# ALVI-Labs/frankenstein

Measured on AMD Instinct MI355X. Metric: neural frames/sec (train fwd+bwd+AdamW, whole job), higher is better.
Workload: dtype bf16; 1 GPU; brainformer-small (6L d=384 6x64 heads, N=6144 tokens) + 2-block perceiver, L1 head; fwd+bwd+clip+AdamW; per_gpu_batch=32, global_batch=32, frames_T=600, electrodes=256, parallelism=dp1, weights=random-init (seed 42)

## Files before the change

### frankenstein_amd/_lib.py

```python
from __future__ import annotations

import ctypes as C
from pathlib import Path

import os

LIB_PATH = Path(os.environ.get("FRANKEN_HIP_LIB") or Path(__file__).resolve().parent / "libfranken_hip.so")

FK_F32, FK_BF16 = 0, 1
MASK_NONE, MASK_CAUSAL, MASK_BLOCK_CAUSAL, MASK_PREFIX, MASK_KEYPAD, MASK_DENSE = 0, 1, 2, 3, 4, 5
NORM_LAYER, NORM_RMS = 0, 1
ATTN_Q_PRESCALED = 1
GEMV_GELU = 1
NT_RING2, NT_RING192, NT_RING128, NT_BIG, NT_GLDS4, NT_GLDS, NT_STAGED = range(7)
NT_ROUTE_F32 = -2
ATTN_FWD_GENERIC, ATTN_FWD_FEWQ, ATTN_FWD_PS, ATTN_FWD_ASM = range(4)
ATTN_DQ_GENERIC, ATTN_DQ_FEWQ, ATTN_DQ_PS, ATTN_DQ_ASM = range(4)
ATTN_DKDV_GENERIC, ATTN_DKDV_PS, ATTN_DKDV_ASM, ATTN_DKDVW_ASM = range(4)

_p, _i64, _int, _f32, _f64, _sz, _u32 = C.c_void_p, C.c_int64, C.c_int, C.c_float, C.c_double, C.c_size_t, C.c_uint32

SIGNATURES = {
    "fk_version": (_int, []),
    "fk_last_error": (C.c_char_p, []),
    "fk_gemm_nt": (_int, [_p, _i64, _p, _i64, _p, _i64, _i64, _i64, _i64, _p, _p, _i64, _i64, _int, _int, _p]),
    "fk_gemv_nt": (_int, [_p, _i64, _p, _i64, _p, _i64, _i64, _i64, _i64, _p, _p, _i64, _p, _p, _f32, _int, _int, _int, _p]),
    "fk_gemm_nt_rope": (_int, [_p, _i64, _p, _i64, _p, _i64, _i64, _i64, _i64, _p, _p, _i64, _i64, _i64, _i64, _i64, _i64, _i64, _int, _p]),
    "fk_gemm_nt_swiglu": (_int, [_p, _i64, _p, _i64, _p, _i64, _p, _i64, _i64, _i64, _i64, _int, _p]),
    "fk_gemm_nt_dswiglu": (_int, [_p, _i64, _p, _i64, _p, _i64, _p, _i64, _i64, _i64, _i64, _int, _p]),
    "fk_mlp_bwd_fused": (_int, [_p, _i64, _p, _i64, _p, _i64, _p, _i64, _p, _i64, _p, _i64, _i64, _i64, _i64, _int, _p]),
    "fk_gemm_nt_route": (_int, [_i64, _i64, _i64, _int, _int, _int, _int]),
    "fk_gemm_tn_route": (_int, [_i64, _i64, _i64, _int, _p, _p]),
    "fk_gemm_tn_workspace_bytes": (_sz, [_i64, _i64, _i64, _int]),
    "fk_gemm_tn": (_int, [_p, _i64, _p, _i64, _p, _i64, _i64, _i64, _i64, _int, _int, _p, _sz, _p]),
    "fk_gemm_tn_swiglu": (_int, [_p, _i64, _p, _i64, _p, _p, _i64, _i64, _i64, _i64, _int, _p, _sz, _p]),
    "fk_colsum_workspace_bytes": (_sz, [_i64, _i64]),
    "fk_colsum": (_int, [_p, _i64, _p, _i64, _i64, _int, _int, _p, _sz, _p]),
    "fk_attn_fwd": (_int, [_p, _p, _p, _p, _p] + [_i64] * 13 + [_int, _i64, _i64, _i64, _p, _p, _f32, _int, _int, _p]),
    "fk_attn_bwd": (_int, [_p] * 10 + [_i64] * 13 + [_int, _i64, _i64, _i64, _p, _p, _f32, _p, _i64, _i64, _int, _int, _p]),
    "fk_attn_fwd_dropout": (_int, [_p, _p, _p, _p, _p] + [_i64] * 13 + [_int, _i64, _i64, _i64, _p, _p, _f32, _int, _f32, _p, _u32, _int, _p]),
    "fk_attn_bwd_dropout": (_int, [_p] * 10 + [_i64] * 13 + [_int, _i64, _i64, _i64, _p, _p, _f32, _p, _i64, _i64, _int, _f32, _p, _u32, _int, _p]),
    "fk_attn_route": (_int, [_i64, _i64, _i64, _int, _int, _i64, _i64, _i64, _int, _int, _int, _p, _p, _p]),
    "fk_dropout": (_int, [_p, _p, _p, _i64, _f32, _p, _u32, _int, _p]),
    "fk_norm_fwd": (_int, [_p, _p, _p, _p, _p, _p, _i64, _i64, _f32, _int, _int, _p]),
    "fk_norm_bwd_workspace_bytes": (_sz, [_i64, _i64]),
    "fk_norm_bwd": (_int, [_p] * 9 + [_i64, _i64, _int, _int, _int, _p, _sz, _p]),
    "fk_rope": (_int, [_p, _i64, _i64, _i64, _i64, _i64, _p, _i64, _i64, _int, _int, _p]),
    "fk_patchify": (_int, [_p, _p, _i64, _i64, _i64, _i64, _i64, _int, _p]),
    "fk_swiglu_fwd": (_int, [_p, _p, _i64, _i64, _int, _p]),
    "fk_swiglu_bwd": (_int, [_p, _p, _p, _i64, _i64, _int, _p]),
    "fk_gelu_fwd": (_int, [_p, _p, _i64, _int, _p]),
    "fk_gelu_bwd": (_int, [_p, _p, _p, _i64, _int, _p]),
    "fk_cast_pack": (_int, [_p, _i64, _p, _i64, _i64, _i64, _int, _int, _p]),
    "fk_cast_pack_rows": (_int, [_p, _i64, _p, _i64, _i64, _i64, _int, _i64, _i64, _i64, _int, _p]),
    "fk_cast_pack_multi": (_int, [_p, _i64, _i64, _int, _p]),
    "fk_cast": (_int, [_p, _int, _p, _int, _i64, _p]),
    "fk_add": (_int, [_p, _p, _p, _i64, _int, _p]),
    "fk_gather_rows": (_int, [_p, _i64, _int, _p, _i64, _p, _i64, _int, _i64, _i64, _i64, _int, _p]),
    "fk_scatter_add_rows": (_int, [_p, _int, _p, _i64, _p, _i64, _i64, _p]),
    "fk_prefix_mask": (_int, [_p, _p, _i64, _p, _p, _i64, _i64, _i64, _p]),
    "fk_copy2d": (_int, [_p, _i64, _p, _i64, _i64, _i64, _int, _p]),
    "fk_attn_combine": (_int, [_p, _p, _p, _p, _i64, _i64, _i64, _i64, _i64, _int, _p]),
    "fk_add2d": (_int, [_p, _i64, _p, _i64, _i64, _i64, _p]),
    "fk_gpt_embed_step": (_int, [_p, _p, _p, _p, _p, _i64, _i64, _i64, _int, _p]),
    "fk_kv_append": (_int, [_p, _p, _p, _i64, _i64, _i64, _int, _p]),
    "fk_attn_decode": (_int, [_p, _i64, _p, _i64, _i64, _p, _i64, _p, _i64, _i64, _i64, _f32, _int, _p]),
    "fk_sample_topk": (_int, [_p, _i64, _i64, _i64, _f32, _i64, _p, _p, _p, _p, _p, _i64, _i64, _p, _p]),
    "fk_attn_decode_beam": (_int, [_p, _i64, _p, _i64, _i64, _p, _i64, _p, _i64, _p, _i64, _i64, _i64, _f32, _int, _p]),
    "fk_beam_topk": (_int, [_p, _i64, _i64, _i64, _f32, _i64, _p, _p, _p]),
    "fk_beam_select": (_int, [_p, _p, _i64, _i64, _i64, _p, _p, _p, _p, _p, _p, _p, _p, _i64, _p, _i64, _p]),
    "fk_attn_decode_beam_grouped": (_int, [_p, _i64, _p, _i64, _i64, _i64, _p, _i64, _p, _i64, _p, _i64, _i64, _i64, _i64, _f32, _int, _int, _p]),
    "fk_beam_select_grouped": (_int, [_p, _p, _i64, _i64, _i64, _i64, _i64, _p, _p, _p, _p, _p, _p, _p, _p, _i64, _p, _i64, _p, _p]),
    "fk_beam_select_eos": (_int, [_p, _p, _i64, _i64, _i64, _i64, _i64, _p, _p, _p, _p, _p, _p, _p, _p, _i64, _p, _i64, _p, _i64, _p, _p, _p, _i64, _p, _p, _p]),
    "fk_beam_backtrack": (_int, [_p, _p, _i64, _i64, _i64, _p, _p, _p, _p, _i64, _p, _i64, _i64, _i64, _i64, _p, _p, _p]),
    "fk_sample_topk_eos": (_int, [_p, _i64, _i64, _i64, _f32, _i64, _p, _p, _p, _p, _p, _i64, _i64, _p, _i64, _p, _p, _p, _p, _p]),
    "fk_sample_topp": (_int, [_p, _i64, _i64, _i64, _f32, _i64, _f32, _p, _p, _p, _p, _p, _i64, _i64, _p, _i64, _p, _p, _p, _p, _p]),
    "fk_logit_rules": (_int, [_p, _i64, _i64, _i64, _f32, _i64, _i64, _i64, _p, _p, _p, _p, _i64, _i64, _i64, _p, _i64, _i64, _int, _p]),
    "fk_im2col1d": (_int, [_p, _p, _i64, _i64, _i64, _i64, _i64, _i64, _int, _p]),
    "fk_col2im1d": (_int, [_p, _p, _i64, _i64, _i64, _i64, _i64, _i64, _int, _p]),
    "fk_elu_fwd": (_int, [_p, _p, _i64, _int, _p]),
    "fk_elu_bwd": (_int, [_p, _p, _p, _i64, _int, _p]),
    "fk_argmax_rows": (_int, [_p, _i64, _p, _i64, _i64, _int, _p]),
    "fk_block_stats_workspace_bytes": (_sz, [_i64, _i64]),
    "fk_block_stats": (_int, [_p, _p, _p, _i64, _i64, _i64, _p, _p, _p, _sz, _p]),
    "fk_zscore_smooth_pad": (_int, [_p, _p, _p, _p, _p, _p, _i64, _i64, _i64, _f64, _p]),
    "fk_gpt_embed_fwd": (_int, [_p, _p, _p, _p, _p, _i64, _i64, _i64, _i64, _i64, _int, _p]),
    "fk_gpt_embed_bwd_wte": (_int, [_p, _p, _p, _i64, _i64, _i64, _i64, _i64, _int, _p]),
    "fk_loss_workspace_bytes": (_sz, [_i64]),
    "fk_l1_loss_fwd": (_int, [_p, _p, _p, _i64, _int, _p, _i64, _int, _p, _sz, _p]),
    "fk_l1_loss_bwd": (_int, [_p, _p, _p, _p, _i64, _int, _p, _i64, _p, _int, _p]),
    "fk_head_ce_workspace_bytes": (_sz, [_i64, _i64]),
    "fk_head_ce_fwd": (_int, [_p, _i64, _p, _i64, _i64, _p, _p, _p, _p, _p, _i64, _i64, _i64, _int, _p, _sz, _p]),
    "fk_head_ce_bwd": (_int, [_p, _i64, _p, _i64, _i64, _p, _p, _p, _p, _p, _p, _i64, _i64, _i64, _p, _i64, _i64, _i64, _i64, _int, _p]),
    "fk_transpose2d": (_int, [_p, _i64, _p, _i64, _i64, _i64, _int, _p]),
    "fk_ce_workspace_bytes": (_sz, [_i64]),
    "fk_ce_loss_fwd": (_int, [_p, _i64, _p, _p, _p, _i64, _i64, _i64, _int, _p, _sz, _p]),
    "fk_ce_loss_bwd": (_int, [_p, _i64, _p, _p, _p, _p, _p, _i64, _i64, _i64, _i64, _int, _p]),
# ... 51 lines not shown
```

### frankenstein_amd/csrc/norm.hip

```cpp
#include <type_traits>

#include "fk_common.h"

namespace {

#ifndef FK_NT_STORES_NORM
#define FK_NT_STORES_NORM 0
#endif
template <typename T> using VIO = VecIO<T, FK_NT_STORES_NORM != 0>;

template <typename T>
__global__ __launch_bounds__(256) void norm_fwd_kernel(const T* x, const float* gamma, const float* beta, T* y,
                                                        float* mean, float* rstd, int64_t rows, int dim, float eps, int kind) {
  constexpr int N = VIO<T>::N;
  const int lane = threadIdx.x & 63, wave = threadIdx.x >> 6;
  const int64_t wstride = (int64_t)gridDim.x * 4;
  for (int64_t row = (int64_t)blockIdx.x * 4 + wave; row < rows; row += wstride) {
    const T* xr = x + row * dim;
    float s = 0.0f;
    float v[N];
    if (kind == FK_NORM_LAYER) {
      for (int c = lane * N; c < dim; c += 64 * N) {
        VIO<T>::load(xr + c, v);
#pragma unroll
        for (int i = 0; i < N; ++i) s += v[i];
      }
    }
    const float mu = kind == FK_NORM_LAYER ? wave_sum(s) / dim : 0.0f;
    float q = 0.0f;
    for (int c = lane * N; c < dim; c += 64 * N) {
      VIO<T>::load(xr + c, v);
#pragma unroll
      for (int i = 0; i < N; ++i) q += (v[i] - mu) * (v[i] - mu);
    }
    const float rs = rsqrtf(wave_sum(q) / dim + eps);
    if (lane == 0) {
      if (mean) mean[row] = mu;
      rstd[row] = rs;
    }
    T* yr = y + row * dim;
    for (int c = lane * N; c < dim; c += 64 * N) {
      VIO<T>::load(xr + c, v);
      float o[N];
#pragma unroll
      for (int i = 0; i < N; ++i) {
        float t = (v[i] - mu) * rs;
        if (kind == FK_NORM_RMS && sizeof(T) == 2) t = (float)(bf16_t)t;
        o[i] = t * gamma[c + i] + (beta ? beta[c + i] : 0.0f);
      }
      VIO<T>::store(yr + c, o);
    }
  }
}

template <int LPR> FK_DEV float row_sum(float v) {
#pragma unroll
  for (int o = LPR / 2; o > 0; o >>= 1) v += __shfl_xor(v, o, 64);
  return v;
}
template <typename T, int LPR, int MAXIT> struct RowFrame {
  static constexpr int N = VIO<T>::N, RPW = 64 / LPR;
  const int l = (threadIdx.x & 63) % LPR, sub = (threadIdx.x & 63) / LPR;
  FK_DEV int col(int it) const { return l * N + it * LPR * N; }
  FK_DEV void load_param(const float* p, bool in, int it, float (&v)[N]) const {
#pragma unroll
    for (int i = 0; i < N; i += 4) {
      const f32x4 p4 = in ? *reinterpret_cast<const f32x4*>(p + col(it) + i) : f32x4{0.0f, 0.0f, 0.0f, 0.0f};
#pragma unroll
      for (int e = 0; e < 4; ++e) v[i + e] = p4[e];
    }
  }
};
template <typename T, int LPR, int MAXIT>
__global__ __launch_bounds__(256) void norm_fwd_fast_kernel(const T* x, const float* gamma, const float* beta, T* y,
                                                             float* mean, float* rstd, int64_t rows, int dim, float eps, int kind) {
  using Frame = RowFrame<T, LPR, MAXIT>;
  constexpr int N = Frame::N, RPW = Frame::RPW;
  const Frame f{};
  const int wave = threadIdx.x >> 6;
  float gm[MAXIT][N], bt[MAXIT][N];
#pragma unroll
  for (int it = 0; it < MAXIT; ++it) {
    const bool in = f.col(it) < dim;
    f.load_param(gamma, in, it, gm[it]);
    f.load_param(beta, in && beta, it, bt[it]);
  }
  const float inv = 1.0f / dim;
  const int64_t stride = (int64_t)gridDim.x * 4 * RPW;
  for (int64_t base = ((int64_t)blockIdx.x * 4 + wave) * RPW; base < rows; base += stride) {
    const int64_t row = base + f.sub;
    const bool ok = row < rows;
    float v[MAXIT][N];
    float s = 0.0f;
#pragma unroll
    for (int it = 0; it < MAXIT; ++it) {
      const int c = f.col(it);
      if (ok && c < dim) VIO<T>::load(x + row * dim + c, v[it]);
      else {
#pragma unroll
        for (int i = 0; i < N; ++i) v[it][i] = 0.0f;
      }
#pragma unroll
      for (int i = 0; i < N; ++i) s += v[it][i];
    }
    const float mu = kind == FK_NORM_LAYER ? row_sum<LPR>(s) * inv : 0.0f;
    float q = 0.0f;
#pragma unroll
    for (int it = 0; it < MAXIT; ++it) {
#pragma unroll
      for (int i = 0; i < N; ++i) {
        const float d = (f.col(it) + i < dim) ? v[it][i] - mu : 0.0f;
        q += d * d;
      }
    }
    const float rs = rsqrtf(row_sum<LPR>(q) * inv + eps);
    if (ok) {
      if (f.l == 0) {
        if (mean) mean[row] = mu;
        rstd[row] = rs;
      }
#pragma unroll
      for (int it = 0; it < MAXIT; ++it) {
        if (f.col(it) < dim) {
          float o[N];
#pragma unroll
          for (int i = 0; i < N; ++i) {
            float t = (v[it][i] - mu) * rs;
            if (kind == FK_NORM_RMS && sizeof(T) == 2) t = (float)(bf16_t)t;
            o[i] = t * gm[it][i] + bt[it][i];
          }
          VIO<T>::store(y + row * dim + f.col(it), o);
        }
      }
    }
  }
}

template <typename T>
__global__ __launch_bounds__(256) void norm_bwd_dx_kernel(const T* dy, const T* x, const float* gamma, const float* mean,
                                                           const float* rstd, const T* dres, T* dx, int64_t rows, int dim, int kind) {
  constexpr int N = VIO<T>::N;
  const int lane = threadIdx.x & 63, wave = threadIdx.x >> 6;
  const int64_t wstride = (int64_t)gridDim.x * 4;
  for (int64_t row = (int64_t)blockIdx.x * 4 + wave; row < rows; row += wstride) {
    const T* xr = x + row * dim;
    const T* gr = dy + row * dim;
    const float mu = (kind == FK_NORM_LAYER) ? mean[row] : 0.0f, rs = rstd[row];
    float s1 = 0.0f, s2 = 0.0f;
    float xv[N], gv[N];
    for (int c = lane * N; c < dim; c += 64 * N) {
      VIO<T>::load(xr + c, xv);
      VIO<T>::load(gr + c, gv);
#pragma unroll
      for (int i = 0; i < N; ++i) {
        const float dg = gv[i] * gamma[c + i];
        s1 += dg;
        s2 += dg * (xv[i] - mu) * rs;
      }
    }
    const float c1 = (kind == FK_NORM_LAYER) ? wave_sum(s1) / dim : 0.0f;
    const float c2 = wave_sum(s2) / dim;
    for (int c = lane * N; c < dim; c += 64 * N) {
      VIO<T>::load(xr + c, xv);
      VIO<T>::load(gr + c, gv);
      float o[N], rv[N];
      if (dres) VIO<T>::load(dres + row * dim + c, rv);
#pragma unroll
      for (int i = 0; i < N; ++i) {
        const float xh = (xv[i] - mu) * rs;
        o[i] = rs * (gv[i] * gamma[c + i] - c1 - xh * c2) + (dres ? rv[i] : 0.0f);
      }
      VIO<T>::store(dx + row * dim + c, o);
    }
  }
}

template <typename T, int LPR, int MAXIT>
__global__ __launch_bounds__(256) void norm_bwd_fused_kernel(const T* dy, const T* x, const float* gamma, const float* mean,
                                                              const float* rstd, const T* dres, T* dx, float* part,
                                                              int64_t rows, int dim, int kind) {
  using Frame = RowFrame<T, LPR, MAXIT>;
  constexpr int N = Frame::N, RPW = Frame::RPW;
  extern __shared__ float red[];
  const Frame f{};
  const int wave = threadIdx.x >> 6;
  float ag[MAXIT][N] = {}, ab[MAXIT][N] = {}, gm[MAXIT][N];
#pragma unroll
  for (int it = 0; it < MAXIT; ++it) f.load_param(gamma, f.col(it) < dim, it, gm[it]);
  const float inv = 1.0f / dim;
  const int64_t stride = (int64_t)gridDim.x * 4 * RPW;
  for (int64_t base = ((int64_t)blockIdx.x * 4 + wave) * RPW; base < rows; base += stride) {
    const int64_t row = base + f.sub;
    const bool ok = row < rows;
    const float mu = (ok && kind == FK_NORM_LAYER) ? mean[row] : 0.0f, rs = ok ? rstd[row] : 0.0f;
    float xv[MAXIT][N], gv[MAXIT][N], rv[MAXIT][N];
    float s1 = 0.0f, s2 = 0.0f;
#pragma unroll
    for (int it = 0; it < MAXIT; ++it) {
      const int c = f.col(it);
      if (ok && c < dim) {
        VIO<T>::load(x + row * dim + c, xv[it]);
        VIO<T>::load(dy + row * dim + c, gv[it]);
        if (dres) VIO<T>::load(dres + row * dim + c, rv[it]);
      } else {
#pragma unroll
        for (int i = 0; i < N; ++i) { xv[it][i] = mu; gv[it][i] = 0.0f; }
      }
#pragma unroll
      for (int i = 0; i < N; ++i) {
        xv[it][i] = (xv[it][i] - mu) * rs;
        const float dg = gv[it][i] * gm[it][i];
        s1 += dg;
        s2 += dg * xv[it][i];
      }
    }
    const float c1 = (kind == FK_NORM_LAYER) ? row_sum<LPR>(s1) * inv : 0.0f;
    const float c2 = row_sum<LPR>(s2) * inv;
#pragma unroll
    for (int it = 0; it < MAXIT; ++it) {
      if (ok && f.col(it) < dim) {
        float o[N];
#pragma unroll
        for (int i = 0; i < N; ++i) {
          o[i] = rs * (gv[it][i] * gm[it][i] - c1 - xv[it][i] * c2) + (dres ? rv[it][i] : 0.0f);
          ag[it][i] += gv[it][i] * xv[it][i];
          ab[it][i] += gv[it][i];
        }
        VIO<T>::store(dx + row * dim + f.col(it), o);
      }
    }
  }
  if (part == nullptr) return;
#pragma unroll
  for (int it = 0; it < MAXIT; ++it)
#pragma unroll
    for (int i = 0; i < N; ++i) {
#pragma unroll
      for (int o = LPR; o < 64; o <<= 1) {
        ag[it][i] += __shfl_xor(ag[it][i], o, 64);
        ab[it][i] += __shfl_xor(ab[it][i], o, 64);
      }
    }
  if (f.sub == 0) {
#pragma unroll
    for (int it = 0; it < MAXIT; ++it) {
      const int c = f.col(it);
      if (c < dim) {
#pragma unroll
        for (int i = 0; i < N; ++i) {
          red[(wave * 2 + 0) * dim + c + i] = ag[it][i];
          red[(wave * 2 + 1) * dim + c + i] = ab[it][i];
        }
      }
    }
  }
  __syncthreads();
  for (int i = threadIdx.x; i < 2 * dim; i += blockDim.x)
    part[(int64_t)blockIdx.x * 2 * dim + i] = red[i] + red[2 * dim + i] + red[4 * dim + i] + red[6 * dim + i];
}
__global__ __launch_bounds__(1024) void norm_bwd_fused_final(const float* part, float* dgamma, float* dbeta, int dim, int nblk, int accumulate) {
  __shared__ float sh[64][17];
  __shared__ float sh2[4][16];
  const int cl = threadIdx.x & 15, sl = threadIdx.x >> 4, c = blockIdx.x * 16 + cl, which = blockIdx.y;
  float s = 0.0f;
  if (c < dim)
    for (int k = sl; k < nblk; k += 64) s += part[((int64_t)k * 2 + which) * dim + c];
  sh[sl][cl] = s;
  __syncthreads();
  if (threadIdx.x < 64) {
    float t = 0.0f;
#pragma unroll
    for (int i = 0; i < 16; ++i) t += sh[sl * 16 + i][cl];
    sh2[sl][cl] = t;
  }
  __syncthreads();
  if (threadIdx.x < 16 && c < dim) {
    float* out = which == 0 ? dgamma : dbeta;
// ... 8 lines not shown
__global__ void norm_bwd_param_partial(const T* dy, const T* x, const float* mean, const float* rstd, float* part,
                                       int64_t rows, int dim, int rows_per_chunk, int kind) {
  const int c = blockIdx.x * blockDim.x + threadIdx.x;
  if (c >= dim) return;
  const int64_t r0 = (int64_t)blockIdx.y * rows_per_chunk, r1 = min(rows, r0 + rows_per_chunk);
  float sg = 0.0f, sb = 0.0f;
  for (int64_t r = r0; r < r1; ++r) {
    const float g = to_f32<T>(dy[r * dim + c]);
    const float mu = (kind == FK_NORM_LAYER) ? mean[r] : 0.0f;
    sg += g * (to_f32<T>(x[r * dim + c]) - mu) * rstd[r];
    sb += g;
  }
  part[((int64_t)blockIdx.y * 2) * dim + c] = sg;
  part[((int64_t)blockIdx.y * 2 + 1) * dim + c] = sb;
}
__global__ void norm_bwd_param_final(const float* part, float* dgamma, float* dbeta, int dim, int nchunk, int accumulate) {
  const int c = blockIdx.x * blockDim.x + threadIdx.x;
  if (c >= dim) return;
  float sg = 0.0f, sb = 0.0f;
  for (int k = 0; k < nchunk; ++k) {
    sg += part[((int64_t)k * 2) * dim + c];
    sb += part[((int64_t)k * 2 + 1) * dim + c];
  }
  if (dgamma) dgamma[c] = accumulate ? dgamma[c] + sg : sg;
  if (dbeta) dbeta[c] = accumulate ? dbeta[c] + sb : sb;
}

int nchunks(int64_t rows) {
  int64_t n = fk_cdiv(rows, 256);
  if (n > 512) n = 512;
  if (n < 1) n = 1;
  return (int)n;
}
int64_t fused_bwd_blocks(int64_t rows) {
  const int64_t n = fk_cdiv(rows, 16);
  return n > 1024 ? 1024 : (n < 1 ? 1 : n);
}

struct Rung { int lpr, maxit; };
template <typename T> struct Ladder;
template <> struct Ladder<bf16_t> { static constexpr Rung rung[] = {{16, 1}, {16, 2}, {16, 3}, {16, 4}, {64, 2}, {64, 4}}; };
template <> struct Ladder<float> { static constexpr Rung rung[] = {{16, 2}, {16, 4}, {16, 6}, {64, 2}, {64, 4}}; };
template <typename T> constexpr int RUNGS = sizeof(Ladder<T>::rung) / sizeof(Rung);
template <typename T, int I> constexpr int64_t RUNG_DIM = (int64_t)Ladder<T>::rung[I].maxit * Ladder<T>::rung[I].lpr * VIO<T>::N;

template <typename T, int I = 0, typename F> bool on_rung(int64_t dim, const F& launch) {
  if constexpr (I < RUNGS<T>) {
    if (dim > RUNG_DIM<T, I>) return on_rung<T, I + 1>(dim, launch);
    launch(std::integral_constant<int, Ladder<T>::rung[I].lpr>{}, std::integral_constant<int, Ladder<T>::rung[I].maxit>{});
    return true;
  }
  return false;
}

}

extern "C" {

int fk_norm_fwd(const void* x, const float* gamma, const float* beta, void* y, float* mean, float* rstd, int64_t rows,
                int64_t dim, float eps, int kind, int dtype, void* stream) {
  FK_DT_CHECK("fk_norm_fwd");
  FK_CHECK_ARG(kind == FK_NORM_LAYER || kind == FK_NORM_RMS, "fk_norm_fwd: bad kind %d", kind);
  const int vec = dtype == FK_BF16 ? 8 : 4;
  FK_CHECK_ARG(rows > 0 && dim > 0 && dim % vec == 0 && dim < (1 << 24), "fk_norm_fwd: dim %lld must be a multiple of %d", (long long)dim, vec);
  FK_CHECK_ARG(x && y && gamma && rstd && (kind == FK_NORM_RMS || mean), "fk_norm_fwd: null pointer");
  FK_CHECK_ARG((((uintptr_t)x | (uintptr_t)y) & 15) == 0, "fk_norm_fwd: x/y must be 16-byte aligned");
  hipStream_t s = (hipStream_t)stream;
  bool done = (((uintptr_t)gamma | (uintptr_t)beta) & 15) == 0;
  if (done)
    FK_BY_DTYPE(dtype, T, done = on_rung<T>(dim, [&](auto lpr, auto maxit) {
      int64_t nbf = fk_cdiv(rows, 4 * (64 / lpr));
      if (nbf > 2048) nbf = 2048;
      hipLaunchKernelGGL((norm_fwd_fast_kernel<T, lpr, maxit>), dim3((unsigned)nbf), dim3(256), 0, s, (const T*)x, gamma, beta, (T*)y, mean, rstd, rows, (int)dim, eps, kind);
    }));
  if (!done) {
    int64_t nb = fk_cdiv(rows, 4);
    if (nb > 8192) nb = 8192;
    FK_BY_DTYPE(dtype, T, hipLaunchKernelGGL(norm_fwd_kernel<T>, dim3((unsigned)nb), dim3(256), 0, s, (const T*)x, gamma, beta, (T*)y, mean, rstd, rows, (int)dim, eps, kind));
  }
  FK_CHECK_LAUNCH("fk_norm_fwd");
  return FK_OK;
}

size_t fk_norm_bwd_workspace_bytes(int64_t rows, int64_t dim) {
  const int64_t nbf = fused_bwd_blocks(rows), n = nbf > nchunks(rows) ? nbf : nchunks(rows);
  return (size_t)n * 2 * dim * sizeof(float);
}

int fk_norm_bwd(const void* dy, const void* x, const float* gamma, const float* mean, const float* rstd, const void* dres,
                void* dx, float* dgamma, float* dbeta, int64_t rows, int64_t dim, int kind, int accumulate, int dtype,
                void* workspace, size_t workspace_bytes, void* stream) {
  FK_DT_CHECK("fk_norm_bwd");
  FK_CHECK_ARG(kind == FK_NORM_LAYER || kind == FK_NORM_RMS, "fk_norm_bwd: bad kind %d", kind);
  const int vec = dtype == FK_BF16 ? 8 : 4;
  FK_CHECK_ARG(rows > 0 && dim > 0 && dim % vec == 0, "fk_norm_bwd: dim %lld must be a multiple of %d", (long long)dim, vec);
  FK_CHECK_ARG(dy && x && gamma && rstd && dx && (kind == FK_NORM_RMS || mean), "fk_norm_bwd: null pointer");
  hipStream_t s = (hipStream_t)stream;
  int64_t top;
  FK_BY_DTYPE(dtype, T, (top = RUNG_DIM<T, RUNGS<T> - 1>));
  const size_t sh = (size_t)8 * dim * sizeof(float);
  const bool fits = dim <= top && sh <= 65536 && ((uintptr_t)gamma & 15) == 0;
  if (fits) {
    const bool want = dgamma || dbeta;
    const int64_t nbf = fused_bwd_blocks(rows);
    if (want) FK_CHECK_ARG(workspace && workspace_bytes >= (size_t)nbf * 2 * dim * sizeof(float), "fk_norm_bwd: workspace too small");
    float* part = want ? (float*)workspace : nullptr;
    FK_BY_DTYPE(dtype, T, on_rung<T>(dim, [&](auto lpr, auto maxit) {
      hipLaunchKernelGGL((norm_bwd_fused_kernel<T, lpr, maxit>), dim3((unsigned)nbf), dim3(256), sh, s, (const T*)dy, (const T*)x, gamma, mean, rstd, (const T*)dres, (T*)dx, part, rows, (int)dim, kind);
    }));
    FK_CHECK_LAUNCH("fk_norm_bwd(fused)");
    if (want) {
      hipLaunchKernelGGL(norm_bwd_fused_final, dim3((unsigned)fk_cdiv(dim, 16), 2), dim3(1024), 0, s, (const float*)part, dgamma, dbeta, (int)dim, (int)nbf, accumulate);
      FK_CHECK_LAUNCH("fk_norm_bwd(fused final)");
    }
    return FK_OK;
  }
  int64_t nb = fk_cdiv(rows, 4);
  if (nb > 8192) nb = 8192;
  FK_BY_DTYPE(dtype, T, hipLaunchKernelGGL(norm_bwd_dx_kernel<T>, dim3((unsigned)nb), dim3(256), 0, s, (const T*)dy, (const T*)x, gamma, mean, rstd, (const T*)dres, (T*)dx, rows, (int)dim, kind));
  FK_CHECK_LAUNCH("fk_norm_bwd(dx)");
  if (dgamma || dbeta) {
    const int nc = nchunks(rows);
    FK_CHECK_ARG(workspace && workspace_bytes >= (size_t)nc * 2 * dim * sizeof(float), "fk_norm_bwd: workspace too small");
    const int rpc = (int)fk_cdiv(rows, nc);
    dim3 grid((unsigned)fk_cdiv(dim, 128), (unsigned)nc);
    FK_BY_DTYPE(dtype, T, hipLaunchKernelGGL(norm_bwd_param_partial<T>, grid, dim3(128), 0, s, (const T*)dy, (const T*)x, mean, rstd, (float*)workspace, rows, (int)dim, rpc, kind));
    FK_CHECK_LAUNCH("fk_norm_bwd(partial)");
    hipLaunchKernelGGL(norm_bwd_param_final, dim3((unsigned)fk_cdiv(dim, 128)), dim3(128), 0, s, (const float*)workspace, dgamma, dbeta, (int)dim, nc, accumulate);
    FK_CHECK_LAUNCH("fk_norm_bwd(final)");
  }
  return FK_OK;
}

}
```

### frankenstein_amd/kernels.py

```python
from __future__ import annotations

import math
from typing import Optional, Tuple

import torch

from . import _lib
from ._lib import FK_BF16, FK_F32, MASK_BLOCK_CAUSAL, MASK_CAUSAL, MASK_DENSE, MASK_KEYPAD, MASK_NONE, MASK_PREFIX, NORM_LAYER, NORM_RMS, ATTN_Q_PRESCALED, call, lib

Tensor = torch.Tensor


TIMERS = None
TIMER_PREFIX = None


class _timed:
    __slots__ = ("name", "ev")

    def __init__(self, name):
        self.name = name

    def __enter__(self):
        self.ev = None
# ... 322 lines not shown
              dq.data_ptr(), dk.data_ptr(), dv.data_ptr(), delta.data_ptr(), B, H, Nq, Nk, D, qb, qr, kb, kr, vb, vr, ob, orr,
              mask.kind, mask.c, mask.q_off, mask.k_off, _ptr(mask.limits), _ptr(mask.qfirst), sc, _ptr(rope_table),
              0 if rope_table is None or rope_table.dim() == 3 else rope_table.stride(0), rope_off,
              ATTN_Q_PRESCALED if q_prescaled else 0)
      if dropout is None:
        call("fk_attn_bwd", *head, fk_dtype(q), _stream())
      else:
        call("fk_attn_bwd_dropout", *head, dropout[0], dropout[1].data_ptr(), dropout[2], fk_dtype(q), _stream())


ATTN_FWD_ROUTE_NAMES = {_lib.ATTN_FWD_GENERIC: "FWD_GENERIC", _lib.ATTN_FWD_FEWQ: "FWD_FEWQ", _lib.ATTN_FWD_PS: "FWD_PS", _lib.ATTN_FWD_ASM: "FWD_ASM"}
ATTN_DQ_ROUTE_NAMES = {_lib.ATTN_DQ_GENERIC: "DQ_GENERIC", _lib.ATTN_DQ_FEWQ: "DQ_FEWQ", _lib.ATTN_DQ_PS: "DQ_PS", _lib.ATTN_DQ_ASM: "DQ_ASM"}
ATTN_DKDV_ROUTE_NAMES = {_lib.ATTN_DKDV_GENERIC: "DKDV_GENERIC", _lib.ATTN_DKDV_PS: "DKDV_PS", _lib.ATTN_DKDV_ASM: "DKDV_ASM", _lib.ATTN_DKDVW_ASM: "DKDVW_ASM"}


def attn_route(Nq: int, Nk: int, D: int, dtype=torch.bfloat16, mask: Mask = NO_MASK, q_prescaled: bool = False, dropout: bool = False,
               rope: bool = False) -> Tuple[int, int, int]:
    import ctypes
    f, q, kv = ctypes.c_int(-1), ctypes.c_int(-1), ctypes.c_int(-1)
    call("fk_attn_route", Nq, Nk, D, fk_dtype(dtype), mask.kind, mask.c, mask.q_off, mask.k_off, ATTN_Q_PRESCALED if q_prescaled else 0,
         int(dropout), int(rope), ctypes.byref(f), ctypes.byref(q), ctypes.byref(kv))
    return f.value, q.value, kv.value


def attn_route_names(*args, **kw) -> Tuple[str, str, str]:
    f, q, kv = attn_route(*args, **kw)
    return ATTN_FWD_ROUTE_NAMES[f], ATTN_DQ_ROUTE_NAMES[q], ATTN_DKDV_ROUTE_NAMES[kv]


def attn_combine(parts: Tensor, lse_parts: Optional[Tensor] = None, want_lse: bool = True):
    B, S, T, H, D = parts.shape
    assert parts.is_contiguous()
    out = torch.empty((B, T, H, D), dtype=parts.dtype, device=parts.device)
    lse = None
    if lse_parts is not None:
        assert lse_parts.dtype == torch.float32 and lse_parts.is_contiguous() and lse_parts.shape == (B, S, H, T)
        lse = torch.empty((B, H, T), dtype=torch.float32, device=parts.device) if want_lse else None
    call("fk_attn_combine", parts.data_ptr(), _ptr(lse_parts), out.data_ptr(), _ptr(lse), B, S, T, H, D, fk_dtype(parts), _stream())
    return out, lse


def norm_fwd(x: Tensor, gamma: Tensor, beta: Optional[Tensor], eps: float, kind: int = NORM_LAYER):
    x2 = _as2d(x)
    assert x2.is_contiguous() and gamma.dtype == torch.float32
    rows, dim = x2.shape
    y = torch.empty_like(x2)
    mean = torch.empty(rows, dtype=torch.float32, device=x.device)
    rstd = torch.empty(rows, dtype=torch.float32, device=x.device)
    call("fk_norm_fwd", x2.data_ptr(), gamma.data_ptr(), _ptr(beta), y.data_ptr(), mean.data_ptr(), rstd.data_ptr(),
         rows, dim, eps, kind, fk_dtype(x), _stream())
    return y.view(x.shape), mean, rstd


def norm_bwd(dy: Tensor, x: Tensor, gamma: Tensor, mean: Tensor, rstd: Tensor, dres: Optional[Tensor] = None,
             kind: int = NORM_LAYER, want_beta: bool = True, dgamma: Optional[Tensor] = None, dbeta: Optional[Tensor] = None,
             accumulate: bool = False):
    x2, dy2 = _as2d(x), _as2d(dy)
    assert x2.is_contiguous() and dy2.is_contiguous() and dy2.dtype == x2.dtype
    rows, dim = x2.shape
    dx = torch.empty_like(x2)
    if dgamma is None:
        assert not accumulate
        dgamma = torch.empty(dim, dtype=torch.float32, device=x.device)
    if dbeta is None and want_beta:
        assert not accumulate
        dbeta = torch.empty(dim, dtype=torch.float32, device=x.device)
    if not want_beta:
        dbeta = None
    for t in (dgamma, dbeta):
        assert t is None or (t.dtype == torch.float32 and t.numel() == dim and t.is_contiguous())
    dres2 = None
    if dres is not None:
        dres2 = _as2d(dres)
        assert dres2.is_contiguous() and dres2.dtype == x2.dtype
    ws, nb = _ws(lib().fk_norm_bwd_workspace_bytes(rows, dim), x.device)
    call("fk_norm_bwd", dy2.data_ptr(), x2.data_ptr(), gamma.data_ptr(), mean.data_ptr(), rstd.data_ptr(), _ptr(dres2),
         dx.data_ptr(), dgamma.data_ptr(), _ptr(dbeta), rows, dim, kind, int(accumulate), fk_dtype(x), _ptr(ws), nb, _stream())
    return dx.view(x.shape), dgamma, dbeta


def rope_(x: Tensor, nheads: int, D: int, table: Tensor, pos_off: int = 0, conj: bool = False) -> Tensor:
    assert x.dim() == 3 and x.stride(2) == 1 and x.stride(0) == x.shape[1] * x.stride(1)
    assert table.dtype == torch.float32 and table.is_contiguous() and table.shape[-1] == 2 and table.shape[-2] == D // 2
    B, T, _ = x.shape
    tbs = 0
    if table.dim() == 4:
        assert table.shape[0] == B
        tbs = table.stride(0)
    assert pos_off >= 0 and pos_off + T <= table.shape[-3], "rope cache shorter than the sequence"
    call("fk_rope", x.data_ptr(), B, T, x.stride(1), nheads, D, table.data_ptr(), tbs, pos_off, int(conj), fk_dtype(x), _stream())
    return x


def patchify(x: Tensor, P: int, ldp: int, dtype: torch.dtype) -> Tensor:
    assert x.dtype == torch.float32 and x.dim() == 3 and x.is_contiguous()
    B, T, Cc = x.shape
    tok = torch.empty((B * (T // P) * Cc, ldp), dtype=dtype, device=x.device)
    call("fk_patchify", x.data_ptr(), tok.data_ptr(), B, T, Cc, P, ldp, fk_dtype(dtype), _stream())
    return tok


def swiglu_fwd(h13: Tensor) -> Tensor:
    assert h13.dim() == 2 and h13.is_contiguous()
    rows, H2 = h13.shape
    g = torch.empty((rows, H2 // 2), dtype=h13.dtype, device=h13.device)
    call("fk_swiglu_fwd", h13.data_ptr(), g.data_ptr(), rows, H2 // 2, fk_dtype(h13), _stream())
# ... 664 lines not shown
```

### include/franken_hip.h

```cpp
#ifndef FRANKEN_HIP_H
#define FRANKEN_HIP_H

#include <stddef.h>
#include <stdint.h>

#ifdef __cplusplus
extern "C" {
#endif

#define FK_VERSION 302

#define FK_OK 0
#define FK_EINVAL (-1)
#define FK_ELAUNCH (-2)
#define FK_EUNSUPPORTED (-3)

enum { FK_F32 = 0, FK_BF16 = 1 };
enum { FK_MASK_NONE = 0, FK_MASK_CAUSAL = 1, FK_MASK_BLOCK_CAUSAL = 2, FK_MASK_PREFIX = 3, FK_MASK_KEYPAD = 4, FK_MASK_DENSE = 5 };
enum { FK_ATTN_Q_PRESCALED = 1 };
enum { FK_NORM_LAYER = 0, FK_NORM_RMS = 1 };
enum { FK_ACT_SWIGLU = 0, FK_ACT_GELU = 1 };
enum { FK_GEMV_GELU = 1 };

int fk_version(void);
// ... 10 lines not shown
                    int64_t rot_cols, int64_t q_cols, int64_t q_table_off, int dtype, void* stream);
int fk_gemm_nt_swiglu(const void* A, int64_t lda, const void* W13, int64_t ldb, void* H13, int64_t ldh, void* G,
                      int64_t ldg, int64_t M, int64_t H, int64_t K, int dtype, void* stream);
int fk_gemm_nt_dswiglu(const void* dY, int64_t lda, const void* W2T, int64_t ldb, const void* H13, int64_t ldh, void* dH13,
                       int64_t lddh, int64_t M, int64_t H, int64_t K, int dtype, void* stream);
int fk_mlp_bwd_fused(const void* dY, int64_t lddy, const void* W2T, int64_t ldw2t, const void* H13, int64_t ldh, const void* W13T,
                     int64_t ldw13t, void* dH13, int64_t lddh, void* dX, int64_t lddx, int64_t M, int64_t H, int64_t D, int dtype,
                     void* stream);
enum { FK_NT_RING2 = 0, FK_NT_RING192 = 1, FK_NT_RING128 = 2, FK_NT_BIG = 3, FK_NT_GLDS4 = 4, FK_NT_GLDS = 5, FK_NT_STAGED = 6 };
#define FK_NT_ROUTE_F32 (-2)
int fk_gemm_nt_route(int64_t M, int64_t N, int64_t K, int dtype, int vec_epi, int mode, int has_rope);
size_t fk_gemm_tn_workspace_bytes(int64_t M, int64_t N1, int64_t N2, int dtype);
int fk_gemm_tn(const void* A, int64_t lda, const void* B, int64_t ldb, float* C, int64_t ldc, int64_t M, int64_t N1,
               int64_t N2, int accumulate, int dtype, void* workspace, size_t workspace_bytes, void* stream);
int fk_gemm_tn_swiglu(const void* A, int64_t lda, const void* B, int64_t ldb, float* d_up, float* d_gate, int64_t ldc, int64_t M,
                      int64_t H, int64_t N2, int dtype, void* workspace, size_t workspace_bytes, void* stream);
int fk_gemm_tn_route(int64_t M, int64_t N1, int64_t N2, int dtype, int* nsplit, int64_t* rows_per_split);
size_t fk_colsum_workspace_bytes(int64_t rows, int64_t cols);
int fk_colsum(const void* X, int64_t ld, float* out, int64_t rows, int64_t cols, int accumulate, int dtype,
              void* workspace, size_t workspace_bytes, void* stream);

int fk_attn_fwd(const void* Q, const void* K, const void* V, void* O, float* LSE, int64_t B, int64_t H, int64_t Nq,
                int64_t Nk, int64_t D, int64_t q_bs, int64_t q_rs, int64_t k_bs, int64_t k_rs, int64_t v_bs,
                int64_t v_rs, int64_t o_bs, int64_t o_rs, int mask_kind, int64_t mask_c, int64_t q_off, int64_t k_off,
                const int32_t* limits, const int32_t* qfirst, float scale, int flags, int dtype, void* stream);
int fk_attn_bwd(const void* Q, const void* K, const void* V, const void* O, const void* dO, const float* LSE,
                void* dQ, void* dK, void* dV, float* delta_ws, int64_t B, int64_t H, int64_t Nq, int64_t Nk, int64_t D,
                int64_t q_bs, int64_t q_rs, int64_t k_bs, int64_t k_rs, int64_t v_bs, int64_t v_rs, int64_t o_bs,
                int64_t o_rs, int mask_kind, int64_t mask_c, int64_t q_off, int64_t k_off, const int32_t* limits,
                const int32_t* qfirst, float scale, const float* rope_table, int64_t rope_bs, int64_t rope_off, int flags,
                int dtype, void* stream);

int fk_attn_fwd_dropout(const void* Q, const void* K, const void* V, void* O, float* LSE, int64_t B, int64_t H, int64_t Nq,
                        int64_t Nk, int64_t D, int64_t q_bs, int64_t q_rs, int64_t k_bs, int64_t k_rs, int64_t v_bs,
                        int64_t v_rs, int64_t o_bs, int64_t o_rs, int mask_kind, int64_t mask_c, int64_t q_off, int64_t k_off,
                        const int32_t* limits, const int32_t* qfirst, float scale, int flags, float drop_p, const uint32_t* drop_seed,
                        uint32_t drop_site, int dtype, void* stream);
int fk_attn_bwd_dropout(const void* Q, const void* K, const void* V, const void* O, const void* dO, const float* LSE,
                        void* dQ, void* dK, void* dV, float* delta_ws, int64_t B, int64_t H, int64_t Nq, int64_t Nk, int64_t D,
                        int64_t q_bs, int64_t q_rs, int64_t k_bs, int64_t k_rs, int64_t v_bs, int64_t v_rs, int64_t o_bs,
                        int64_t o_rs, int mask_kind, int64_t mask_c, int64_t q_off, int64_t k_off, const int32_t* limits,
                        const int32_t* qfirst, float scale, const float* rope_table, int64_t rope_bs, int64_t rope_off, int flags,
                        float drop_p, const uint32_t* drop_seed, uint32_t drop_site, int dtype, void* stream);
enum { FK_ATTN_FWD_GENERIC = 0, FK_ATTN_FWD_FEWQ = 1, FK_ATTN_FWD_PS = 2, FK_ATTN_FWD_ASM = 3 };
enum { FK_ATTN_DQ_GENERIC = 0, FK_ATTN_DQ_FEWQ = 1, FK_ATTN_DQ_PS = 2, FK_ATTN_DQ_ASM = 3 };
enum { FK_ATTN_DKDV_GENERIC = 0, FK_ATTN_DKDV_PS = 1, FK_ATTN_DKDV_ASM = 2, FK_ATTN_DKDVW_ASM = 3 };
int fk_attn_route(int64_t Nq, int64_t Nk, int64_t D, int dtype, int mask_kind, int64_t mask_c, int64_t q_off, int64_t k_off, int flags,
                  int has_dropout, int has_rope, int* fwd, int* dq, int* dkdv);

int fk_dropout(const void* x, const void* res, void* y, int64_t n, float p, const uint32_t* seed, uint32_t site, int dtype, void* stream);

int fk_norm_fwd(const void* x, const float* gamma, const float* beta, void* y, float* mean, float* rstd,
                int64_t rows, int64_t dim, float eps, int kind, int dtype, void* stream);
size_t fk_norm_bwd_workspace_bytes(int64_t rows, int64_t dim);
int fk_norm_bwd(const void* dy, const void* x, const float* gamma, const float* mean, const float* rstd,
                const void* dres, void* dx, float* dgamma, float* dbeta, int64_t rows, int64_t dim, int kind,
                int accumulate, int dtype, void* workspace, size_t workspace_bytes, void* stream);

int fk_rope(void* x, int64_t B, int64_t T, int64_t ld, int64_t nheads, int64_t D, const float* table, int64_t table_bs,
            int64_t pos_off, int conj, int dtype, void* stream);

int fk_patchify(const float* x, void* tok, int64_t B, int64_t T, int64_t C, int64_t P, int64_t ldp, int dtype,
                void* stream);

int fk_swiglu_fwd(const void* h13, void* g, int64_t rows, int64_t H, int dtype, void* stream);
int fk_swiglu_bwd(const void* h13, const void* dg, void* dh13, int64_t rows, int64_t H, int dtype, void* stream);
int fk_gelu_fwd(const void* x, void* y, int64_t n, int dtype, void* stream);
int fk_gelu_bwd(const void* x, const void* dy, void* dx, int64_t n, int dtype, void* stream);

int fk_cast_pack(const float* src, int64_t lds, void* dst, int64_t ldd, int64_t rows, int64_t cols, int transpose,
                 int dtype, void* stream);
int fk_cast_pack_rows(const float* src, int64_t lds, void* dst, int64_t ldd, int64_t rows, int64_t cols, int transpose,
                      int64_t rblk, int64_t rstride, int64_t roff, int dtype, void* stream);
typedef struct fk_pack_job {
  const float* src; void* dst; int64_t lds, ldd;
  int32_t rows, cols, transpose, rblk, rstride, roff;
  int64_t chunk_begin;
} fk_pack_job;
int fk_cast_pack_multi(const fk_pack_job* jobs, int64_t njobs, int64_t total_chunks, int dtype, void* stream);
int fk_cast(const void* src, int src_dtype, void* dst, int dst_dtype, int64_t n, void* stream);
int fk_add(const void* a, const void* b, void* y, int64_t n, int dtype, void* stream);

int fk_attn_combine(const void* parts, const float* lse_parts, void* out, float* lse_out, int64_t B, int64_t S, int64_t T, int64_t H,
                    int64_t D, int dtype, void* stream);

int fk_gpt_embed_step(const int64_t* idx, const float* wte, const float* wpe, const int32_t* pos, void* out, int64_t B, int64_t dim,
                      int64_t vocab, int dtype, void* stream);
int fk_kv_append(const void* qkv, void* kv, const int32_t* pos, int64_t B, int64_t d, int64_t tmax, int dtype, void* stream);
int fk_attn_decode(const void* q, int64_t q_bs, const void* kv, int64_t kv_bs, int64_t kv_rs, void* out, int64_t o_bs, const int32_t* pos,
                   int64_t B, int64_t H, int64_t D, float scale, int dtype, void* stream);
int fk_sample_topk(const float* logits, int64_t ld, int64_t B, int64_t V, float temperature, int64_t top_k, const uint64_t* seed,
                   int64_t* step, int32_t* pos_inc, int64_t* cur, int64_t* out, int64_t out_ld, int64_t out_cols, uint32_t* ticket,
                   void* stream);

int fk_attn_decode_beam(const void* q, int64_t q_bs, const void* kv, int64_t kv_bs, int64_t kv_rs, const int32_t* anc, int64_t anc_ld, void* out,
                        int64_t o_bs, const int32_t* pos, int64_t W, int64_t H, int64_t D, float scale, int dtype, void* stream);
int fk_beam_topk(const float* logits, int64_t ld, int64_t R, int64_t V, float temperature, int64_t k, float* top_lp, int64_t* top_id, void* stream);
int fk_beam_select(const float* top_lp, const int64_t* top_id, int64_t row_stride, int64_t W, int64_t k, float* scores, const uint64_t* seed,
                   int64_t* step, const int32_t* pos, int32_t* pos_inc, int64_t* cur, int32_t* parent_log, int64_t* tok_log, int64_t log_rows,
                   int32_t* anc, int64_t anc_ld, void* stream);

int fk_attn_decode_beam_grouped(const void* qkv, int64_t q_bs, void* kv, int64_t kv_bs, int64_t kv_rs, int64_t tmax, const int32_t* anc, int64_t anc_ld,
                                void* out, int64_t o_bs, const int32_t* pos, int64_t S, int64_t W, int64_t H, int64_t D, float scale, int append, int dtype,
                                void* stream);
int fk_beam_select_grouped(const float* top_lp, const int64_t* top_id, int64_t row_stride, int64_t group_stride, int64_t S, int64_t W, int64_t k,
                           float* scores, const uint64_t* seed, int64_t* step, const int32_t* pos, int32_t* pos_inc, int64_t* cur, int32_t* parent_log,
// ... 105 lines not shown
```

Baseline: 400,900 frames/s.

## Software-prefetch next row in norm kernels and size grid by occupancy

The fast LayerNorm/RMSNorm forward and fused backward kernels now issue packed loads for the next row-group before working on the current one, so global memory latency overlaps with compute. Launch bounds now request a minimum occupancy computed from the register footprint, and the forward grid is capped at CUs times waves rather than a fixed 2048. A query entry point, fk_norm_grid, is added to report the chosen grid. The prefetch buffers add register pressure, which could lower occupancy or cause spills for wide rows.

```diff
diff --git a/frankenstein_amd/_lib.py b/frankenstein_amd/_lib.py
--- a/frankenstein_amd/_lib.py
+++ b/frankenstein_amd/_lib.py
@@ -43,6 +43,7 @@
     "fk_attn_route": (_int, [_i64, _i64, _i64, _int, _int, _i64, _i64, _i64, _int, _int, _int, _p, _p, _p]),
     "fk_dropout": (_int, [_p, _p, _p, _i64, _f32, _p, _u32, _int, _p]),
     "fk_norm_fwd": (_int, [_p, _p, _p, _p, _p, _p, _i64, _i64, _f32, _int, _int, _p]),
+    "fk_norm_grid": (_int, [_i64, _i64, _int, _p, _p]),
     "fk_norm_bwd_workspace_bytes": (_sz, [_i64, _i64]),
     "fk_norm_bwd": (_int, [_p] * 9 + [_i64, _i64, _int, _int, _int, _p, _sz, _p]),
     "fk_rope": (_int, [_p, _i64, _i64, _i64, _i64, _i64, _p, _i64, _i64, _int, _int, _p]),
diff --git a/frankenstein_amd/csrc/norm.hip b/frankenstein_amd/csrc/norm.hip
--- a/frankenstein_amd/csrc/norm.hip
+++ b/frankenstein_amd/csrc/norm.hip
@@ -71,8 +71,26 @@
     }
   }
 };
+template <typename T> struct PackedVec;
+template <> struct PackedVec<bf16_t> { using V = bf16x8; };
+template <> struct PackedVec<float> { using V = f32x4; };
+template <typename T> using PV = u32x4;
+template <typename T> FK_DEV PV<T> load_packed(const T* p) { return *reinterpret_cast<const u32x4*>(p); }
+template <typename T, int N> FK_DEV void widen(const PV<T>& p, float (&v)[N]) {
+  const typename PackedVec<T>::V a = __builtin_bit_cast(typename PackedVec<T>::V, p);
+#pragma unroll
+  for (int i = 0; i < N; ++i) v[i] = (float)a[i];
+}
+
+constexpr int FK_CUS = 256;
+template <typename T, int MAXIT> constexpr int ROW_FLOATS = MAXIT * VIO<T>::N;
+template <typename T, int MAXIT> constexpr int PACKED_REGS = ROW_FLOATS<T, MAXIT> * (int)sizeof(T) / 4;
+template <typename T, int MAXIT> constexpr int FWD_WAVES = 3 * ROW_FLOATS<T, MAXIT> + PACKED_REGS<T, MAXIT> <= 88 ? 4 : 3;
+template <typename T, int MAXIT> constexpr int BWD_REGS = 5 * ROW_FLOATS<T, MAXIT> + 4 * PACKED_REGS<T, MAXIT>;
+template <typename T, int MAXIT> constexpr int BWD_WAVES = BWD_REGS<T, MAXIT> <= 72 ? 4 : BWD_REGS<T, MAXIT> <= 100 ? 3 : BWD_REGS<T, MAXIT> <= 200 ? 2 : 1;
+
 template <typename T, int LPR, int MAXIT>
-__global__ __launch_bounds__(256) void norm_fwd_fast_kernel(const T* x, const float* gamma, const float* beta, T* y,
+__global__ __launch_bounds__(256, (FWD_WAVES<T, MAXIT>)) void norm_fwd_fast_kernel(const T* x, const float* gamma, const float* beta, T* y,
                                                              float* mean, float* rstd, int64_t rows, int dim, float eps, int kind) {
   using Frame = RowFrame<T, LPR, MAXIT>;
   constexpr int N = Frame::N, RPW = Frame::RPW;
@@ -87,19 +105,28 @@
   }
   const float inv = 1.0f / dim;
   const int64_t stride = (int64_t)gridDim.x * 4 * RPW;
-  for (int64_t base = ((int64_t)blockIdx.x * 4 + wave) * RPW; base < rows; base += stride) {
+  int64_t base = ((int64_t)blockIdx.x * 4 + wave) * RPW;
+  PV<T> nx[MAXIT];
+  auto request = [&](int64_t b) __attribute__((always_inline)) {
+    const int64_t r = b + f.sub;
+#pragma unroll
+    for (int it = 0; it < MAXIT; ++it) {
+      const int c = f.col(it);
+      if (r < rows && c < dim) nx[it] = load_packed<T>(x + r * dim + c);
+      else nx[it] = PV<T>{};
+    }
+  };
+  if (base < rows) request(base);
+  for (; base < rows; base += stride) {
     const int64_t row = base + f.sub;
     const bool ok = row < rows;
     float v[MAXIT][N];
     float s = 0.0f;
 #pragma unroll
-    for (int it = 0; it < MAXIT; ++it) {
-      const int c = f.col(it);
-      if (ok && c < dim) VIO<T>::load(x + row * dim + c, v[it]);
-      else {
-#pragma unroll
-        for (int i = 0; i < N; ++i) v[it][i] = 0.0f;
-      }
+    for (int it = 0; it < MAXIT; ++it) widen<T>(nx[it], v[it]);
+    if (base + stride < rows) request(base + stride);
+#pragma unroll
+    for (int it = 0; it < MAXIT; ++it) {
 #pragma unroll
       for (int i = 0; i < N; ++i) s += v[it][i];
     }
@@ -176,7 +203,7 @@
 }
 
 template <typename T, int LPR, int MAXIT>
-__global__ __launch_bounds__(256) void norm_bwd_fused_kernel(const T* dy, const T* x, const float* gamma, const float* mean,
+__global__ __launch_bounds__(256, (BWD_WAVES<T, MAXIT>)) void norm_bwd_fused_kernel(const T* dy, const T* x, const float* gamma, const float* mean,
                                                               const float* rstd, const T* dres, T* dx, float* part,
                                                               int64_t rows, int dim, int kind) {
   using Frame = RowFrame<T, LPR, MAXIT>;
@@ -189,26 +216,50 @@
   for (int it = 0; it < MAXIT; ++it) f.load_param(gamma, f.col(it) < dim, it, gm[it]);
   const float inv = 1.0f / dim;
   const int64_t stride = (int64_t)gridDim.x * 4 * RPW;
-  for (int64_t base = ((int64_t)blockIdx.x * 4 + wave) * RPW; base < rows; base += stride) {
+  int64_t base = ((int64_t)blockIdx.x * 4 + wave) * RPW;
+  PV<T> nx[MAXIT], ng[MAXIT], nr[MAXIT];
+  float nmu = 0.0f, nrs = 0.0f;
+  auto request = [&](int64_t b) __attribute__((always_inline)) {
+    const int64_t r = b + f.sub;
+    const bool rok = r < rows;
+    nmu = (rok && kind == FK_NORM_LAYER) ? mean[r] : 0.0f;
+    nrs = rok ? rstd[r] : 0.0f;
+#pragma unroll
+    for (int it = 0; it < MAXIT; ++it) {
+      const int c = f.col(it);
+      if (rok && c < dim) {
+        nx[it] = load_packed<T>(x + r * dim + c);
+        ng[it] = load_packed<T>(dy + r * dim + c);
+        if (dres) nr[it] = load_packed<T>(dres + r * dim + c);
+        else nr[it] = PV<T>{};
+      } else {
+        nx[it] = PV<T>{};
+        ng[it] = PV<T>{};
+        nr[it] = PV<T>{};
+      }
+    }
+  };
+  if (base < rows) request(base);
+  for (; base < rows; base += stride) {
     const int64_t row = base + f.sub;
     const bool ok = row < rows;
-    const float mu = (ok && kind == FK_NORM_LAYER) ? mean[row] : 0.0f, rs = ok ? rstd[row] : 0.0f;
-    float xv[MAXIT][N], gv[MAXIT][N], rv[MAXIT][N];
+    const float mu = nmu, rs = nrs;
+    float xv[MAXIT][N], gv[MAXIT][N];
+    PV<T> pr[MAXIT];
+#pragma unroll
+    for (int it = 0; it < MAXIT; ++it) {
+      widen<T>(nx[it], xv[it]);
+      widen<T>(ng[it], gv[it]);
+      pr[it] = nr[it];
+    }
+    if (base + stride < rows) request(base + stride);
     float s1 = 0.0f, s2 = 0.0f;
 #pragma unroll
     for (int it = 0; it < MAXIT; ++it) {
-      const int c = f.col(it);
-      if (ok && c < dim) {
-        VIO<T>::load(x + row * dim + c, xv[it]);
-        VIO<T>::load(dy + row * dim + c, gv[it]);
-        if (dres) VIO<T>::load(dres + row * dim + c, rv[it]);
-      } else {
-#pragma unroll
-        for (int i = 0; i < N; ++i) { xv[it][i] = mu; gv[it][i] = 0.0f; }
-      }
+      const bool in = ok && f.col(it) < dim;
 #pragma unroll
       for (int i = 0; i < N; ++i) {
-        xv[it][i] = (xv[it][i] - mu) * rs;
+        xv[it][i] = ((in ? xv[it][i] : mu) - mu) * rs;
         const float dg = gv[it][i] * gm[it][i];
         s1 += dg;
         s2 += dg * xv[it][i];
@@ -219,10 +270,11 @@
 #pragma unroll
     for (int it = 0; it < MAXIT; ++it) {
       if (ok && f.col(it) < dim) {
-        float o[N];
+        float rv[N], o[N];
+        if (dres) widen<T>(pr[it], rv);
 #pragma unroll
         for (int i = 0; i < N; ++i) {
-          o[i] = rs * (gv[it][i] * gm[it][i] - c1 - xv[it][i] * c2) + (dres ? rv[it][i] : 0.0f);
+          o[i] = rs * (gv[it][i] * gm[it][i] - c1 - xv[it][i] * c2) + (dres ? rv[i] : 0.0f);
           ag[it][i] += gv[it][i] * xv[it][i];
           ab[it][i] += gv[it][i];
         }
@@ -337,6 +389,14 @@
   }
   return false;
 }
+template <typename T, int LPR, int MAXIT> int64_t fwd_blocks(int64_t rows) {
+  const int64_t n = fk_cdiv(rows, 4 * (64 / LPR)), cap = (int64_t)FK_CUS * FWD_WAVES<T, MAXIT>;
+  return n > cap ? cap : n;
+}
+int64_t generic_blocks(int64_t rows) {
+  const int64_t nb = fk_cdiv(rows, 4);
+  return nb > 8192 ? 8192 : nb;
+}
 
 }
 
@@ -354,17 +414,31 @@
   bool done = (((uintptr_t)gamma | (uintptr_t)beta) & 15) == 0;
   if (done)
     FK_BY_DTYPE(dtype, T, done = on_rung<T>(dim, [&](auto lpr, auto maxit) {
-      int64_t nbf = fk_cdiv(rows, 4 * (64 / lpr));
-      if (nbf > 2048) nbf = 2048;
+      const int64_t nbf = fwd_blocks<T, lpr, maxit>(rows);
       hipLaunchKernelGGL((norm_fwd_fast_kernel<T, lpr, maxit>), dim3((unsigned)nbf), dim3(256), 0, s, (const T*)x, gamma, beta, (T*)y, mean, rstd, rows, (int)dim, eps, kind);
     }));
   if (!done) {
-    int64_t nb = fk_cdiv(rows, 4);
-    if (nb > 8192) nb = 8192;
+    const int64_t nb = generic_blocks(rows);
     FK_BY_DTYPE(dtype, T, hipLaunchKernelGGL(norm_fwd_kernel<T>, dim3((unsigned)nb), dim3(256), 0, s, (const T*)x, gamma, beta, (T*)y, mean, rstd, rows, (int)dim, eps, kind));
   }
   FK_CHECK_LAUNCH("fk_norm_fwd");
   return FK_OK;
+}
+
+int fk_norm_grid(int64_t rows, int64_t dim, int dtype, int64_t* fwd_blocks_out, int64_t* bwd_blocks_out) {
+  FK_DT_CHECK("fk_norm_grid");
+  const int vec = dtype == FK_BF16 ? 8 : 4;
+  FK_CHECK_ARG(rows > 0 && dim > 0 && dim % vec == 0 && dim < (1 << 24), "fk_norm_grid: dim %lld must be a multiple of %d", (long long)dim, vec);
+  int lanes = 0;
+  int64_t nf = generic_blocks(rows), nb = generic_blocks(rows);
+  FK_BY_DTYPE(dtype, T, on_rung<T>(dim, [&](auto lpr, auto maxit) {
+    lanes = lpr;
+    nf = fwd_blocks<T, lpr, maxit>(rows);
+    nb = fused_bwd_blocks(rows);
+  }));
+  if (fwd_blocks_out) *fwd_blocks_out = nf;
+  if (bwd_blocks_out) *bwd_blocks_out = nb;
+  return lanes;
 }
 
 size_t fk_norm_bwd_workspace_bytes(int64_t rows, int64_t dim) {
@@ -400,8 +474,7 @@
     }
     return FK_OK;
   }
-  int64_t nb = fk_cdiv(rows, 4);
-  if (nb > 8192) nb = 8192;
+  const int64_t nb = generic_blocks(rows);
   FK_BY_DTYPE(dtype, T, hipLaunchKernelGGL(norm_bwd_dx_kernel<T>, dim3((unsigned)nb), dim3(256), 0, s, (const T*)dy, (const T*)x, gamma, mean, rstd, (const T*)dres, (T*)dx, rows, (int)dim, kind));
   FK_CHECK_LAUNCH("fk_norm_bwd(dx)");
   if (dgamma || dbeta) {
diff --git a/frankenstein_amd/kernels.py b/frankenstein_amd/kernels.py
--- a/frankenstein_amd/kernels.py
+++ b/frankenstein_amd/kernels.py
@@ -398,6 +398,15 @@
     return y.view(x.shape), mean, rstd
 
 
+def norm_grid(rows: int, dim: int, dtype=torch.bfloat16) -> Tuple[int, int, int]:
+    import ctypes
+    nf, nb = ctypes.c_int64(0), ctypes.c_int64(0)
+    r = lib().fk_norm_grid(rows, dim, fk_dtype(dtype), ctypes.byref(nf), ctypes.byref(nb))
+    if r < 0:
+        _lib.check(r, "fk_norm_grid")
+    return r, nf.value, nb.value
+
+
 def norm_bwd(dy: Tensor, x: Tensor, gamma: Tensor, mean: Tensor, rstd: Tensor, dres: Optional[Tensor] = None,
              kind: int = NORM_LAYER, want_beta: bool = True, dgamma: Optional[Tensor] = None, dbeta: Optional[Tensor] = None,
              accumulate: bool = False):
diff --git a/include/franken_hip.h b/include/franken_hip.h
--- a/include/franken_hip.h
+++ b/include/franken_hip.h
@@ -86,6 +86,7 @@
 
 int fk_norm_fwd(const void* x, const float* gamma, const float* beta, void* y, float* mean, float* rstd,
                 int64_t rows, int64_t dim, float eps, int kind, int dtype, void* stream);
+int fk_norm_grid(int64_t rows, int64_t dim, int dtype, int64_t* fwd_blocks, int64_t* bwd_blocks);
 size_t fk_norm_bwd_workspace_bytes(int64_t rows, int64_t dim);
 int fk_norm_bwd(const void* dy, const void* x, const float* gamma, const float* mean, const float* rstd,
                 const void* dres, void* dx, float* dgamma, float* dbeta, int64_t rows, int64_t dim, int kind,
```

Measured after the change: 403,200 frames/s (median of 6 runs). Within noise of the previous version (+0.6%).
